# USCbiostats/bayesnetworks

Hardware: NVIDIA B200
Metric: edge_proposals_scored_per_sec (higher is better)
Workload: dtype f64

## Files before the change

### bayesnetworks_b200/csrc/chain_core.cuh

```cuda
#pragma once

#include "bn_common.cuh"
#include "rng_core.cuh"
#include "score_core.cuh"

namespace bn {

constexpr int WIN = 32;
constexpr int REPLAY_POS = 256;

constexpr int REC_LEN_MASK = 0xff;
constexpr int REC_TYPE = 1 << 8;
constexpr int REC_CYC = 1 << 9;
constexpr int REC_OVF = 1 << 10;
constexpr int REC_AG = 1 << 11;
constexpr int REC_ACC = 1 << 12;
constexpr int REC_NPD = 1 << 13;
constexpr int REC_FULLMANY = 1 << 14;
constexpr int REC_STALE = 1 << 15;
constexpr int REC_KK_SHIFT = 16;
constexpr int REC_NOSCORE = 1 << 23;
constexpr int REC_CLOSE = 1 << 24;
constexpr int WALK_STOP = 3 << 20;
constexpr int WALK_OVF = WALK_STOP | (1 << 24);
constexpr int WALK_STALE = WALK_STOP | (1 << 25);
constexpr int WALK_END = WALK_STOP | (1 << 26);

struct ChainParams {
  int P, max_par, W, Ws, n_samples;
  const double* C;
  int64_t ldc;
  const double* diag;
  ScoreConsts sc;
  const uint8_t* node_type;
  const uint8_t* sim_edge;
  int n_sim_edges;
  double phi, omega;
  int initial_network, drop, n_iter, output_every;
  int trace_capacity, moves_capacity;
  const int* prior_par;
  const int* prior_npar;
  int prior_stride;
  int g_chunks, g_lpr, g_rpp;
};

struct PipeLink;

struct ChainStart {
  int64_t iter;
  int valid;
  int te_m;
  int acc_add, acc_del;
};

struct ChainMem {
  int* par;
  int* npar;
  int* born;
  double* base;
  double* fac;
  double* rowbuf;
  uint32_t* anc;
  uint32_t* haspar;
  int* hp_list;
  int* scratch;
  volatile int* helper;
  int* t_iter; int* t_changed; int* t_movetype; double* t_gll;
  int* t_add; int* t_del; int* t_fn; int* t_fp;
  int* moves;
  int* edge_freq;
  double* dscore;
  int* npar_freq;
  int* npar_since;
  uint32_t* nver = nullptr;
  PipeLink* pipe = nullptr;
  int pipe_rank = 0;
  int pipe_debug = 0;
  const int* start_par = nullptr;
  const int* start_npar = nullptr;
  const ChainStart* start = nullptr;
  const double* base_in = nullptr;
};

struct ChainScalars {
  int64_t iter;
  int64_t read_pos;
  int valid;
  int te_m;
  int te_true, agree_true, n_haspar;
  int proposed[3], reject[3];
  int n_rows, n_moves, n_nonpd;
  int64_t valid_iters;
  int lane_prop[3], lane_rej[3], lane_nonpd, lane_valid;
  int64_t lane_bytes;
  int acc_add, acc_del;
  int gll_ok; double gll;
  int64_t alg_bytes;
  long long cyc[12];
  long long slots_sim;
  int win;
  int windows;
  int need_full;
  int anc_changed;
  int next_log;
  int status;
  int64_t pw_cur, pw_out_pos;
  int pw_out_seq, pw_out;
  int pw_seen;
  int pw_waits, pw_discards, pw_rebuilds;
  long long pw_cyc[6];
};

struct WindowSlots {
  int child[WIN], parent[WIN], pos[WIN], kk[WIN];
  int te_m[WIN], fp_m[WIN], fn_m[WIN];
  int64_t pos_after[WIN];
  double u_acc[WIN], new_score[WIN];
  signed char type[WIN], valid[WIN], do_check[WIN], accept[WIN], nonpd[WIN];
  int t_c[REPLAY_POS], t_j[REPLAY_POS], t_e[REPLAY_POS];
  int t_rec[REPLAY_POS];
  double t_score[REPLAY_POS];
  uint32_t t_full[REPLAY_POS];
  double t_lu[REPLAY_POS];
  int t_walk[2 * REPLAY_POS];
  int s_k[WIN];
};

BN_HD long long cycle_now() {
#if defined(__CUDA_ARCH__) && defined(BN_PHASE_CYCLES)
  return clock64();
#else
  return 0;
#endif
}

#if defined(BN_EMU_STATS) && !defined(__CUDA_ARCH__)
struct EmuStats { long del_total, del_trivial, del_desc, del_rounds, del_rows_eval, del_lost_bits, add_total, add_trivial, add_desc; };
inline EmuStats& emu_stats() { static EmuStats s = {}; return s; }
#define BN_STAT(x) x
#else
#define BN_STAT(x)
#endif

BN_HD bool test_bit(const uint32_t* row, int b) { return (row[b >> 5] >> (b & 31)) & 1u; }

BN_HD double prior_value(double phi, double omega, int dist, int total_edges) {
  return sub_rn(mul_rn(-phi, (double)dist), mul_rn(omega, (double)total_edges));
}

BN_HD int rank_below(const uint32_t* bits, int c) {
  const int l = Warp::lane(), cw = c >> 5;
  int cnt = 0;
  for (int w = l; w <= cw; w += Warp::NL) {
    uint32_t word = bits[w];
    if (w == cw) word &= (1u << (c & 31)) - 1u;
    cnt += popc32(word);
  }
  return Warp::sum(cnt);
}

BN_HD void hp_insert(ChainMem& m, int n_before, int c) {
  const int l = Warp::lane();
  const int idx = rank_below(m.haspar, c);
  for (int hi = n_before; hi > idx; hi -= Warp::NL) {
    const int i = hi - 1 - l;
    const int v = (i >= idx) ? m.hp_list[i] : 0;
    Warp::sync();
    if (i >= idx) m.hp_list[i + 1] = v;
    Warp::sync();
  }
  if (l == 0) m.hp_list[idx] = c;
  Warp::sync();
}
BN_HD void hp_remove(ChainMem& m, int n_before, int c) {
  const int l = Warp::lane();
  const int idx = rank_below(m.haspar, c);
  for (int lo = idx; lo < n_before - 1; lo += Warp::NL) {
    const int i = lo + l;
    const int v = (i < n_before - 1) ? m.hp_list[i + 1] : 0;
    Warp::sync();
    if (i < n_before - 1) m.hp_list[i] = v;
    Warp::sync();
  }
}

struct alignas(16) U4 { uint32_t x, y, z, w; };
BN_HD U4 or4(U4 a, U4 b) { U4 r; r.x = a.x | b.x; r.y = a.y | b.y; r.z = a.z | b.z; r.w = a.w | b.w; return r; }
BN_HD U4 andn4(U4 a, U4 b) { U4 r; r.x = a.x & ~b.x; r.y = a.y & ~b.y; r.z = a.z & ~b.z; r.w = a.w & ~b.w; return r; }
BN_HD U4 and4(U4 a, U4 b) { U4 r; r.x = a.x & b.x; r.y = a.y & b.y; r.z = a.z & b.z; r.w = a.w & b.w; return r; }
BN_HD bool nz4(U4 a) { return (a.x | a.y | a.z | a.w) != 0u; }
BN_HD bool ne4(U4 a, U4 b) { return ((a.x ^ b.x) | (a.y ^ b.y) | (a.z ^ b.z) | (a.w ^ b.w)) != 0u; }
BN_HD int popc4(U4 a) { return popc32(a.x) + popc32(a.y) + popc32(a.z) + popc32(a.w); }
BN_HD U4 with_bit(U4 v, int b) {
  const uint32_t m = 1u << (b & 31);
  const int w = b >> 5;
  v.x |= (w == 0) ? m : 0u; v.y |= (w == 1) ? m : 0u; v.z |= (w == 2) ? m : 0u; v.w |= (w == 3) ? m : 0u;
  return v;
}

struct RowGeom { int chunks, lpr, rpp; };
BN_HD void set_row_geom(ChainParams& p) {
  p.g_chunks = (p.W + 3) / 4;
  p.g_lpr = 1;
  while (p.g_lpr < p.g_chunks && p.g_lpr < Warp::NL) p.g_lpr <<= 1;
  p.g_rpp = Warp::NL / p.g_lpr;
}
BN_HD RowGeom row_geom(const ChainParams& p) {
  RowGeom g;
  g.chunks = p.g_chunks; g.lpr = p.g_lpr; g.rpp = p.g_rpp;
  return g;
}

BN_HD int group_sum(int v, int lpr) {
#if defined(__CUDA_ARCH__)
  for (int o = 1; o < lpr; o <<= 1) v += __shfl_xor_sync(0xffffffffu, v, o);
#else
  (void)lpr;
#endif
  return v;
}

BN_HD int atomic_fetch_inc(int* p) {
#if defined(__CUDA_ARCH__)
  return atomicAdd(p, 1);
#else
  return (*p)++;
#endif
}

BN_HD uint32_t atomic_or_u32(uint32_t* p, uint32_t v) {
#if defined(__CUDA_ARCH__)
  return atomicOr(p, v);
#else
  const uint32_t o = *p; *p = o | v; return o;
#endif
}

BN_HD int rows_per_part(int P, int nparts, int nl) {
  const int nblk = (P + nl - 1) / nl;
  return (nblk + nparts - 1) / nparts * nl;
}
BN_HD int scratch_words(int P, int nparts, int nl) {
  const int W = (P + 31) / 32;
  const int n = 2 * rows_per_part(P, nparts, nl) * nparts + 4 + (W + 3) / 4 * 4 + 3 * W + 4 + 1 + (W + 3) / 4 + 28;
  return (n + 3) / 4 * 4;
}

BN_HD int collect_desc_part(const ChainParams& p, const ChainMem& m, int c, int include_self, int* list,
                            int part, int nparts) {
  const int l = Warp::lane();
  const uint32_t Ws = (uint32_t)p.Ws, cb = (uint32_t)c & 31u;
  const uint32_t* col = m.anc + (c >> 5);
  const uint32_t lt = (1u << l) - 1u;
  int n = 0;
  const int step = nparts * Warp::NL;
  for (int d0 = part * Warp::NL; d0 < p.P; d0 += 4 * step) {
    int d[4], flag[4];
#pragma unroll
    for (int t = 0; t < 4; t++) {
      d[t] = d0 + t * step + l;
      flag[t] = 0;
      if (d[t] < p.P) flag[t] = ((col[(uint32_t)d[t] * Ws] >> cb) & 1u) & ((include_self || d[t] != c) ? 1u : 0u);
    }
#pragma unroll
    for (int t = 0; t < 4; t++) {
      const uint32_t mask = Warp::ballot(flag[t]);
      if (flag[t]) list[n + popc32(mask & lt)] = d[t];
      n += popc32(mask);
    }
  }
  Warp::sync();
  return n;
}

BN_HD void anc_add_part(const ChainParams& p, const ChainMem& m, int j, int c, int* list, int part, int nparts) {
  const RowGeom g = row_geom(p);
  const int l = Warp::lane(), sub = l / g.lpr, li = l % g.lpr;
  const int n = collect_desc_part(p, m, c, 1, list, part, nparts);
  BN_STAT(emu_stats().add_desc += n;)
  const U4* aj = (const U4*)(m.anc + (uint32_t)j * (uint32_t)p.Ws);
  if (g.chunks == 8 && Warp::NL == 32) {
    const int sub8 = l >> 3, li8 = l & 7;
    const U4 a = aj[li8];
    for (int r0 = sub8; r0 < n; r0 += 16) {
      U4* ad[4];
      U4 v[4];
#pragma unroll
      for (int t = 0; t < 4; t++) {
        const int r = (r0 + 4 * t < n) ? r0 + 4 * t : r0;
        ad[t] = (U4*)(m.anc + (uint32_t)list[r] * (uint32_t)p.Ws) + li8;
      }
#pragma unroll
      for (int t = 0; t < 4; t++) v[t] = *ad[t];
#pragma unroll
      for (int t = 0; t < 4; t++) *ad[t] = or4(v[t], a);
    }
  } else if (g.chunks <= g.lpr) {
    U4 a = {0u, 0u, 0u, 0u};
    if (li < g.chunks) {
      a = aj[li];
    }
    for (int r0 = 0; r0 < n; r0 += 4 * g.rpp) {
      U4* ad[4];
      U4 v[4];
#pragma unroll
      for (int t = 0; t < 4; t++) {
        const int r = r0 + t * g.rpp + sub;
        ad[t] = (r < n && li < g.chunks) ? (U4*)(m.anc + (uint32_t)list[r] * (uint32_t)p.Ws) + li : nullptr;
      }
#pragma unroll
      for (int t = 0; t < 4; t++) if (ad[t]) v[t] = *ad[t];
#pragma unroll
      for (int t = 0; t < 4; t++) if (ad[t]) *ad[t] = or4(v[t], a);
    }
  } else {
    for (int r0 = 0; r0 < n; r0 += g.rpp) {
      const int r = r0 + sub;
      if (r < n) {
        U4* ad = (U4*)(m.anc + (int64_t)list[r] * p.Ws);
        for (int ch = li; ch < g.chunks; ch += g.lpr) {
          ad[ch] = or4(ad[ch], aj[ch]);
        }
      }
    }
  }
  Warp::sync();
}

constexpr int HELPER_WARPS = 7;
enum { HELPER_EXIT = 0, HELPER_ANC_ADD = 1, HELPER_RECORDS = 2, HELPER_REPAIR = 3, HELPER_ANC_DEL = 4,
       HELPER_FILL_WH = 5, HELPER_PIPE_COPY = 6, HELPER_REPAIR_BATCH = 7 };
constexpr int HELPER_WORDS = 12;
#if defined(__CUDACC__)
__device__ __forceinline__ void cta_bar(int id) {
  asm volatile("bar.sync %0, %1;" ::"r"(id), "r"((HELPER_WARPS + 1) * 32) : "memory");
}
#endif
constexpr int PIPE_WIN = HELPER_WARPS * 32;
constexpr int PIPE_MQ = 64;
constexpr int PIPE_LOG = 128;
struct PipeLink {
  unsigned long long req;
  int req_exit;
  int pad0;
  unsigned long long rdy;
  int mq_tail;
  int pad1;
  alignas(16) int mq[PIPE_MQ][4];
  int log[PIPE_LOG];
};
constexpr int PIPE_MAX_NODES = 2048;
constexpr int LOG_NODE = 0xffffff, LOG_UNFULL = 1 << 24, LOG_ANC = 1 << 25, LOG_HP = 1 << 26;

#if defined(__CUDACC__)
__device__ __forceinline__ uint32_t smem_addr(const void* p) { return (uint32_t)__cvta_generic_to_shared(p); }
__device__ __forceinline__ uint32_t peer_addr(const void* p, int rank) {
  uint32_t r;
  asm volatile("mapa.shared::cluster.u32 %0, %1, %2;" : "=r"(r) : "r"(smem_addr(p)), "r"(rank));
  return r;
}
__device__ __forceinline__ void st_peer(uint32_t a, int v) {
  asm volatile("st.relaxed.cluster.shared::cluster.b32 [%0], %1;" ::"r"(a), "r"(v) : "memory");
}
__device__ __forceinline__ void st_peer64(uint32_t a, unsigned long long v) {
  asm volatile("st.relaxed.cluster.shared::cluster.b64 [%0], %1;" ::"r"(a), "l"(v) : "memory");
}
__device__ __forceinline__ void st_peer128(uint32_t a, int x, int y, int z, int w) {
  asm volatile("st.shared::cluster.v4.b32 [%0], {%1, %2, %3, %4};" ::"r"(a), "r"(x), "r"(y), "r"(z), "r"(w) : "memory");
}
__device__ __forceinline__ int ld_poll(const int* p) {
  int v;
  asm volatile("ld.volatile.shared.b32 %0, [%1];" : "=r"(v) : "r"(smem_addr(p)) : "memory");
  return v;
}
__device__ __forceinline__ unsigned long long ld_poll64(const unsigned long long* p) {
  unsigned long long v;
  asm volatile("ld.volatile.shared.b64 %0, [%1];" : "=l"(v) : "r"(smem_addr(p)) : "memory");
  return v;
}
__device__ __forceinline__ void ld_poll128(const int* p, int& x, int& y, int& z, int& w) {
  asm volatile("ld.volatile.shared.v4.b32 {%0, %1, %2, %3}, [%4];" : "=r"(x), "=r"(y), "=r"(z), "=r"(w) : "r"(smem_addr(p)) : "memory");
}
__device__ __forceinline__ int ld_peer(uint32_t a) {
  int v;
  asm volatile("ld.shared::cluster.b32 %0, [%1];" : "=r"(v) : "r"(a) : "memory");
  return v;
}
__device__ __forceinline__ long long ld_peer64(uint32_t a) {
  long long v;
  asm volatile("ld.shared::cluster.b64 %0, [%1];" : "=l"(v) : "r"(a) : "memory");
  return v;
}
__device__ __forceinline__ void cluster_sync_all() {
  asm volatile("barrier.cluster.arrive.release.aligned;\n\tbarrier.cluster.wait.acquire.aligned;" ::: "memory");
}

__device__ __forceinline__ void pipe_publish(const ChainMem& m, int n, int type, int c, int j, int del, int ag,
                                             double score, int flags) {
  PipeLink* lk = m.pipe;
  for (long long spins = 0; n - ld_poll(&lk->mq_tail) >= PIPE_MQ; spins++)
    if (spins > (1ll << 27)) { lk->pad1 = 92; break; }
  const long long sb = __double_as_longlong(score);
  st_peer128(peer_addr(&lk->mq[n % PIPE_MQ][0], 1), n + 1,
             c | (j << 11) | ((type - 1) << 22) | (del << 23) | (ag << 26) | ((n + 1) << 27),
             (int)(sb & 0xffffffffll), (int)(sb >> 32));
  lk->log[n % PIPE_LOG] = c | flags;
}
#endif

BN_HD void team_sync(const ChainMem& m) {
#if defined(__CUDA_ARCH__)
  if (m.helper) { cta_bar(3); return; }
#endif
  (void)m;
  Warp::sync();
}

BN_HD void anc_after_add(const ChainParams& p, ChainMem& m, int j, int c, int& m_anc_changed) {
  {
    const RowGeom g = row_geom(p);
    const U4* aj = (const U4*)(m.anc + (uint32_t)j * (uint32_t)p.Ws);
    const U4* ac = (const U4*)(m.anc + (uint32_t)c * (uint32_t)p.Ws);
    int news = 0;
    for (int ch = Warp::lane(); ch < g.chunks; ch += Warp::NL) news |= nz4(andn4(aj[ch], ac[ch])) ? 1 : 0;
    BN_STAT(emu_stats().add_total++;)
    if (Warp::ballot(news) == 0u) { BN_STAT(emu_stats().add_trivial++;) m_anc_changed = 0; return; }
  }
  m_anc_changed = 1;
#if defined(__CUDA_ARCH__)
  if (m.helper) {
    if (Warp::lane() == 0) { m.helper[8] = j; m.helper[9] = c; m.helper[0] = HELPER_ANC_ADD; }
    Warp::sync();
    cta_bar(1);
    if (!m.pipe) anc_add_part(p, m, j, c, m.scratch, 0, HELPER_WARPS + 1);
    cta_bar(2);
    return;
  }
#else
  anc_add_part(p, m, j, c, m.scratch, 0, 1);
#endif
}


struct Par8 { int q[8]; };
BN_HD Par8 load_par8(const ChainParams& p, const ChainMem& m, int d) {
  Par8 r;
  const int* pd = m.par + (int64_t)d * p.max_par;
  if (p.max_par == 8) {
    const U4 a = ((const U4*)pd)[0], b = ((const U4*)pd)[1];
    r.q[0] = (int)a.x; r.q[1] = (int)a.y; r.q[2] = (int)a.z; r.q[3] = (int)a.w;
    r.q[4] = (int)b.x; r.q[5] = (int)b.y; r.q[6] = (int)b.z; r.q[7] = (int)b.w;
  } else {
#pragma unroll
    for (int e = 0; e < 8; e++) r.q[e] = (e < p.max_par) ? pd[e] : -1;
  }
  return r;
}

struct DelLayout { int* lists; U4* L; uint32_t* dirty; volatile int* flags; int* nzc; int per; };
BN_HD DelLayout del_layout(const ChainParams& p, const ChainMem& m, int nparts) {
  DelLayout d;
  d.per = rows_per_part(p.P, nparts, Warp::NL);
  int off = (2 * d.per * nparts + 3) / 4 * 4;
  d.lists = m.scratch;
  d.L = (U4*)(m.scratch + off);
  off += (p.W + 3) / 4 * 4;
  d.dirty = (uint32_t*)(m.scratch + off);
  d.flags = (volatile int*)(d.dirty + 3 * p.W);
  d.nzc = (int*)(d.dirty + 3 * p.W + 4);
  return d;
}

BN_HD int anc_del_team(const ChainParams& p, const ChainMem& m, int c, int part, int nparts, long long* dbg = nullptr) {
  const int l = Warp::lane(), W = p.W, MP = p.max_par;
  const DelLayout lay = del_layout(p, m, nparts);
  int* list = lay.lists + (part < 0 ? 0 : part) * 2 * lay.per;
  int* list2 = list + lay.per;
  const long long td0 = cycle_now();
  const int n = part < 0 ? 0 : collect_desc_part(p, m, c, 0, list, part, nparts);
  BN_STAT(emu_stats().del_desc += n;)
  const uint32_t lt = (l == 31) ? 0x7fffffffu : ((1u << l) - 1u);
  const int nnz = lay.nzc[0];
  int lpr = 1;
  while (lpr < nnz && lpr < Warp::NL) lpr <<= 1;
  const int rpp = Warp::NL / lpr, sub = l / lpr, li = l % lpr;
  const uint32_t gm = (lpr >= 32 ? 0xffffffffu : ((1u << lpr) - 1u)) << (sub * lpr);
  for (int r0 = 0; r0 < n; r0 += rpp) {
    const int r = r0 + sub;
    if (r < n) {
      U4* ad = (U4*)(m.anc + (uint32_t)list[r] * (uint32_t)p.Ws);
      for (int t = li; t < nnz; t += lpr) {
        const int ch = lay.nzc[1 + t];
        ad[ch] = andn4(ad[ch], lay.L[ch]);
      }
    }
  }
  const long long td1 = cycle_now();
  team_sync(m);
  const long long td2 = cycle_now();
  if (dbg) { dbg[6] += td1 - td0; dbg[7] += td2 - td1; }
  int rounds_done = 0;
  for (int round = 0;; round++) {
    const long long tr0 = cycle_now();
    const uint32_t* dprev = lay.dirty + (round % 3) * W;
    uint32_t* dnext = lay.dirty + ((round + 1) % 3) * W;
    if (part <= 0 && (part < 0 || !m.pipe)) {
      uint32_t* dclr = lay.dirty + ((round + 2) % 3) * W;
      for (int w = l; w < W; w += Warp::NL) dclr[w] = 0u;
      if (l == 0) lay.flags[(round + 2) % 4] = 0;
    }
    const int* rows = list;
    int nt = n;
    if (round > 0) {
      rows = list2;
      nt = 0;
      for (int i0 = 0; i0 < n; i0 += Warp::NL) {
        const int i = i0 + l;
        const int d = (i < n) ? list[i] : -1;
        int touched = 0;
        if (d >= 0) {
          if (MP <= 8) {
            const Par8 pq = load_par8(p, m, d);
#pragma unroll
            for (int e = 0; e < 8; e++)
              if (pq.q[e] >= 0) touched |= (dprev[pq.q[e] >> 5] >> (pq.q[e] & 31)) & 1u;
          } else {
            const int kd = m.npar[d];
            const int* pd = m.par + (int64_t)d * MP;
            for (int e = 0; e < kd; e++) {
              const int q = pd[e];
              touched |= (dprev[q >> 5] >> (q & 31)) & 1u;
            }
          }
        }
        const uint32_t mask = Warp::ballot(touched);
        if (touched) list2[nt + popc32(mask & lt)] = d;
        nt += popc32(mask);
      }
      Warp::sync();
    }
    int any = 0;
    BN_STAT(emu_stats().del_rounds++; emu_stats().del_rows_eval += nt;)
    for (int r0 = 0; r0 < nt; r0 += rpp) {
      const int r = r0 + sub;
      int changed = 0, d = 0;
      if (r < nt) {
        d = rows[r];
        U4* ad = (U4*)(m.anc + (uint32_t)d * (uint32_t)p.Ws);
        for (int t = li; t < nnz; t += lpr) {
          const int ch = lay.nzc[1 + t];
          const U4 Lc = lay.L[ch];
          U4 v = {0u, 0u, 0u, 0u};
          if (MP <= 8) {
            const Par8 pq = load_par8(p, m, d);
#pragma unroll
            for (int e = 0; e < 8; e++) {
              const int q = pq.q[e];
              if (q >= 0) v = or4(v, ((const U4*)(m.anc + (uint32_t)q * (uint32_t)p.Ws))[ch]);
            }
          } else {
            const int kd = m.npar[d];
            const int* pd = m.par + (int64_t)d * MP;
            for (int e = 0; e < kd; e++) {
              const int q = pd[e];
              v = or4(v, ((const U4*)(m.anc + (int64_t)q * p.Ws))[ch]);
            }
          }
          const U4 cur = ad[ch];
          const U4 gain = andn4(and4(v, Lc), cur);
          if (nz4(gain)) { ad[ch] = or4(cur, gain); changed = 1; }
        }
      }
      const uint32_t mask = Warp::ballot(changed);
      if (r < nt && li == 0 && (mask & gm)) atomic_or_u32(&dnext[d >> 5], 1u << (d & 31));
      any |= (mask != 0u);
      Warp::sync();
    }
    if (any && l == 0) lay.flags[round % 4] = 1;
    const long long tr1 = cycle_now();
    team_sync(m);
    if (dbg) { dbg[8] += tr1 - tr0; dbg[11] += cycle_now() - tr1; }
    rounds_done++;
    if (lay.flags[round % 4] == 0) break;
  }
  return rounds_done;
}

BN_HD void anc_after_delete(const ChainParams& p, ChainMem& m, int c, int& m_anc_changed, long long* dbg = nullptr) {
  const RowGeom g = row_geom(p);
  const int l = Warp::lane();
  int nparts = 1;
#if defined(__CUDA_ARCH__)
  if (m.helper) nparts = m.pipe ? HELPER_WARPS : HELPER_WARPS + 1;
#endif
  const DelLayout lay = del_layout(p, m, nparts);
  {
    U4* ac = (U4*)(m.anc + (int64_t)c * p.Ws);
    const int* pc = m.par + (int64_t)c * p.max_par;
    const int kc = m.npar[c];
    int changed = 0;
    for (int ch = l; ch < g.chunks; ch += Warp::NL) {
      U4 v = {0u, 0u, 0u, 0u};
      if (ch == (c >> 7)) v = with_bit(v, c & 127);
      for (int e = 0; e < kc; e++) {
        const int q = pc[e];
        v = or4(v, ((const U4*)(m.anc + (int64_t)q * p.Ws))[ch]);
      }
      const U4 lost = andn4(ac[ch], v);
      lay.L[ch] = lost;
      if (nz4(lost)) { ac[ch] = v; changed = 1; }
    }
    BN_STAT(emu_stats().del_total++;)
    if (Warp::ballot(changed) == 0u) { BN_STAT(emu_stats().del_trivial++;) m_anc_changed = 0; return; }
  }
  m_anc_changed = 1;
  BN_STAT(for (int ch = 0; ch < g.chunks; ch++) emu_stats().del_lost_bits += popc4(lay.L[ch]);)
  for (int w = l; w < 3 * p.W + 4; w += Warp::NL) lay.dirty[w] = 0u;
  Warp::sync();
  {
    const uint32_t lt = (l == 31) ? 0x7fffffffu : ((1u << l) - 1u);
    int nnz = 0;
    for (int ch0 = 0; ch0 < g.chunks; ch0 += Warp::NL) {
      const int ch = ch0 + l;
      const int nz = (ch < g.chunks) && nz4(lay.L[ch]);
      const uint32_t mask = Warp::ballot(nz);
      if (nz) lay.nzc[1 + nnz + popc32(mask & lt)] = ch;
      nnz += popc32(mask);
    }
    if (l == 0) lay.nzc[0] = nnz;
    Warp::sync();
  }
#if defined(__CUDA_ARCH__)
  if (m.helper) {
    if (l == 0) { m.helper[9] = c; m.helper[0] = HELPER_ANC_DEL; }
    Warp::sync();
    cta_bar(1);
    anc_del_team(p, m, c, m.pipe ? -1 : 0, nparts, dbg);
    cta_bar(2);
    return;
  }
#else
  anc_del_team(p, m, c, 0, 1);
#endif
}

BN_HD void anc_reset(const ChainParams& p, ChainMem& m) {
  const int l = Warp::lane();
  for (int64_t i = l; i < (int64_t)p.P * p.Ws; i += Warp::NL) m.anc[i] = 0u;
  Warp::sync();
  for (int d = l; d < p.P; d += Warp::NL) m.anc[(int64_t)d * p.Ws + (d >> 5)] = 1u << (d & 31);
  Warp::sync();
}

BN_HD void anc_build_all(const ChainParams& p, ChainMem& m) {
  const RowGeom g = row_geom(p);
  const int l = Warp::lane(), P = p.P;
  anc_reset(p, m);
  for (int round = 0; round <= P; round++) {
    int changed = 0;
    for (int d = 0; d < P; d++) {
      const int kd = m.npar[d];
      if (kd == 0) continue;
      U4* ad = (U4*)(m.anc + (int64_t)d * p.Ws);
      const int* pd = m.par + (int64_t)d * p.max_par;
      for (int ch = l; ch < g.chunks; ch += Warp::NL) {
        U4 v = {0u, 0u, 0u, 0u};
        if (ch == (d >> 7)) v = with_bit(v, d & 127);
        for (int e = 0; e < kd; e++) {
          const int q = pd[e];
          v = or4(v, ((const U4*)(m.anc + (int64_t)q * p.Ws))[ch]);
        }
        if (ne4(v, ad[ch])) { ad[ch] = v; changed = 1; }
      }
      Warp::sync();
    }
    if (Warp::ballot(changed) == 0u) break;
  }
  Warp::sync();
}

template <int KMAX>
BN_HD double factor_current(const ChainParams& p, const ChainMem& m, int c) {
  const int MP = p.max_par, k = m.npar[c];
  double* F = m.fac + (int64_t)c * fac_stride(fac_mp(MP));
  if (k <= 8) {
    Parents8 S;
    const Par8 q = load_par8(p, m, c);
#pragma unroll
    for (int e = 0; e < 8; e++) S.s[e] = q.q[e];
    return factor_node8(p.C, p.ldc, c, S, k, p.sc, F, fac_mp(MP));
  }
  return factor_node(p.C, p.ldc, c, m.par + (int64_t)c * MP, k, p.sc, F, fac_mp(MP));
}

template <int KMAX>
BN_HD int64_t random_start(const ChainParams& p, ChainMem& m, RngStream& rng) {
  const int P = p.P, MP = p.max_par;
  int64_t pos = 0;
  int anc_changed = 0;
  for (int c = 0; c < P; c++) {
    if (p.node_type[c] == 1) continue;
    if (pos >= rng.gen_hi) rng_top_up(rng, pos);
    const int want = (int)(MP * rng.ubuf[pos & (RNG_CAP - 1)]);
    pos++;
    for (int slot = 0; slot < want; slot++) {
      int found = -1;
      for (int tries = 0; tries < 100 && found < 0; tries++) {
        if (pos >= rng.gen_hi) rng_top_up(rng, pos);
        const int j = (int)(P * rng.ubuf[pos & (RNG_CAP - 1)]);
        pos++;
        int ok = (j != c && p.node_type[j] != 2 && !test_bit(m.anc + (int64_t)j * p.Ws, c));
        for (int e = 0; e < slot; e++) if (m.par[(int64_t)c * MP + e] == j) ok = 0;
        if (ok) found = j;
      }
      if (found < 0) break;
      Warp::sync();
      if (Warp::lane() == 0) { m.par[(int64_t)c * MP + slot] = found; m.npar[c] = slot + 1; }
      Warp::sync();
      anc_after_add(p, m, found, c, anc_changed);
    }
  }
  return pos;
}

template <int KMAX>
BN_HD void chain_init(const ChainParams& p, ChainMem& m, ChainScalars& s, RngStream& rng) {
  const int l = Warp::lane(), P = p.P, MP = p.max_par;
  const bool given = m.start_par != nullptr;
  const int64_t it0 = m.start ? m.start->iter : 0;
  const int counted_from = (m.start && it0 > p.drop) ? (int)it0 : p.drop;
  for (int64_t i = l; i < (int64_t)P * MP; i += Warp::NL) {
    const int c = (int)(i / MP), e = (int)(i % MP);
    m.par[i] = given ? m.start_par[i]
                     : (p.initial_network == 0 && e < p.prior_npar[c]) ? p.prior_par[(int64_t)c * p.prior_stride + e] : -1;
    if (m.born) m.born[i] = counted_from;
  }
  if (m.npar_freq)
    for (int i = l; i < P; i += Warp::NL) m.npar_since[i] = counted_from;
  for (int i = l; i < P; i += Warp::NL) m.npar[i] = given ? m.start_npar[i] : (p.initial_network == 0) ? p.prior_npar[i] : 0;
  for (int w = l; w < p.W; w += Warp::NL) m.haspar[w] = 0u;
  if (m.nver)
    for (int i = l; i < P; i += Warp::NL) m.nver[i] = 0u;
  Warp::sync();
  int64_t start_pos = 0;
  const bool random = !given && p.initial_network == 1;
  if (random) {
    anc_reset(p, m);
    start_pos = random_start<KMAX>(p, m, rng);
  }
  if (l == 0) {
    int te = 0, ag = 0, nh = 0;
    for (int c = 0; c < P; c++) {
      const int k = m.npar[c];
      if (k) { m.haspar[c >> 5] |= 1u << (c & 31); m.hp_list[nh] = c; nh++; }
      for (int e = 0; e < k; e++) {
        te++;
        if (p.sim_edge[(int64_t)m.par[(int64_t)c * MP + e] + (int64_t)c * P]) ag++;
      }
    }
    s.te_true = te; s.agree_true = ag; s.n_haspar = nh;
  }
  s.te_true = Warp::shfl(s.te_true, 0);
  s.agree_true = Warp::shfl(s.agree_true, 0);
  s.n_haspar = Warp::shfl(s.n_haspar, 0);
  Warp::sync();
  if (random) {  }
  else if (s.te_true > 0) anc_build_all(p, m);
  else anc_reset(p, m);
  s.n_nonpd = 0;
  for (int c = l; c < P; c += Warp::NL) {
    if (m.base_in) {
      m.base[c] = m.base_in[c];
    } else if (KMAX <= 8) {
      Parents8 S;
      const int k = m.npar[c];
#pragma unroll
      for (int e = 0; e < 8; e++) S.s[e] = (e < k) ? m.par[(int64_t)c * MP + e] : c;
      m.base[c] = score_set8(p.C, p.ldc, c, S, k, p.n_samples);
    } else {
      m.base[c] = factor_current<KMAX>(p, m, c);
    }
  }
  Warp::sync();
  s.iter = it0; s.read_pos = start_pos;
  s.valid = m.start ? m.start->valid : 1;
  s.te_m = m.start ? m.start->te_m : 0;
  for (int t = 0; t < 3; t++) { s.proposed[t] = 0; s.reject[t] = 0; s.lane_prop[t] = 0; s.lane_rej[t] = 0; }
  s.lane_nonpd = 0; s.lane_valid = 0; s.lane_bytes = 0;
  s.acc_add = m.start ? m.start->acc_add : 0; s.acc_del = m.start ? m.start->acc_del : 0;
  s.n_rows = 0; s.n_moves = 0; s.valid_iters = 0; s.alg_bytes = 0;
  s.gll_ok = 0; s.gll = 0.0;
// ... 631 lines not shown
template <int KMAX, bool PIPE = false>
BN_HD void team_records(const ChainParams& p, const ChainMem& m, const RoundCtx& rc, const double* ubuf,
                        WindowSlots& ws) {
#if defined(__CUDA_ARCH__)
  if (m.helper) {
    helper_post(m, HELPER_RECORDS, rc);
    cta_bar(1);
    if constexpr (!PIPE) build_record<KMAX>(p, m, rc, ubuf, ws, Warp::lane());
    cta_bar(2);
    return;
  }
#else
  for (int slot = Warp::lane(); slot < REPLAY_POS; slot += Warp::NL) build_record<KMAX>(p, m, rc, ubuf, ws, slot);
  Warp::sync();
#endif
}

BN_HD void team_repair(const ChainParams& p, const ChainMem& m, WindowSlots& ws, int c, int unfull, int retest,
                       int from) {
#if defined(__CUDA_ARCH__)
  if (m.helper) {
    if (Warp::lane() == 0) {
      m.helper[8] = from; m.helper[9] = c; m.helper[11] = unfull; m.helper[7] = retest;
      m.helper[0] = HELPER_REPAIR;
    }
    Warp::sync();
    cta_bar(1);
    if (!m.pipe) repair_record(p, m, ws, Warp::lane(), c, unfull, retest, from);
    cta_bar(2);
  }
#else
  for (int slot = Warp::lane(); slot < REPLAY_POS; slot += Warp::NL)
    repair_record(p, m, ws, slot, c, unfull, retest, from);
  Warp::sync();
#endif
}

BN_HD void write_row_vals(const ChainParams& p, ChainMem& m, ChainScalars& s, int64_t it, int child,
                          int type, int fn, int fp, int additions, int deletions) {
  if (!s.gll_ok) { s.gll = sum_base(p, m); s.gll_ok = 1; }
  if (s.n_rows < p.trace_capacity) {
    if (Warp::lane() == 0) {
      const int r = s.n_rows;
      m.t_iter[r] = (int)it;
      m.t_changed[r] = child;
      m.t_movetype[r] = type;
      m.t_gll[r] = s.gll;
      m.t_add[r] = additions;
      m.t_del[r] = deletions;
      m.t_fn[r] = fn;
      m.t_fp[r] = fp;
    }
    s.n_rows++;
  }
}
BN_HD void write_row(const ChainParams& p, ChainMem& m, ChainScalars& s, int64_t it,
                     const WindowSlots& ws, int i, int additions, int deletions) {
  write_row_vals(p, m, s, it, ws.child[i], ws.type[i], ws.fn_m[i], ws.fp_m[i], additions, deletions);
}

template <int KMAX>
BN_HD void apply_move_vals(const ChainParams& p, ChainMem& m, ChainScalars& s, int64_t it, int type, int c,
                           int j, int del, double new_score, int ag, const double* newrow) {
  const int MP = p.max_par, l = Warp::lane();
#if defined(__CUDA_ARCH__)
  if (m.pipe) {
    const int kk0 = m.npar[c];
    bool bad = (type == 1) ? (kk0 >= MP) : (del < 0 || del >= kk0 || m.par[(int64_t)c * MP + del] != j);
    if (type == 1) for (int e = 0; e < kk0 && e < MP; e++) bad |= m.par[(int64_t)c * MP + e] == j;
    if (bad) { s.status = 95; return; }
  }
#endif
  int* pc = m.par + (int64_t)c * MP;
  int* bc = m.born ? m.born + (int64_t)c * MP : nullptr;
  const int k = m.npar[c];
  double* F = KMAX > 8 ? m.fac + (int64_t)c * fac_stride(fac_mp(MP)) : nullptr;
#if defined(__CUDA_ARCH__)
  D2 rv, rd, rr;
  rv.x = rv.y = rd.x = rd.y = rr.x = rr.y = 0.0;
  if (KMAX > 8 && type == 1 && newrow) {
    if (2 * l < k) rv = ld2_l2(newrow + 2 * l);
    rd = ld2_l2(newrow + row_tail(fac_mp(MP)));
    rr = ld2_l2(newrow + row_tail(fac_mp(MP)) + 2);
  }
#endif
  const long long tq0 = cycle_now();
  const int64_t first_counted = (it > p.drop) ? it : p.drop;
#if defined(__CUDA_ARCH__)
  const bool publish = m.pipe && m.pipe_rank == 0 && m.pipe_debug != 2;
  const long long tp0 = cycle_now();
  if (publish && l == 0)
    pipe_publish(m, s.n_moves, type, c, j, type == 2 ? del : 0, ag, new_score,
                 ((type == 2 && k == MP) ? LOG_UNFULL : 0) | ((type == 1 ? k == 0 : k == 1) ? LOG_HP : 0));
  s.pw_cyc[5] += cycle_now() - tp0;
#endif
  Warp::sync();
  if (l == 0 && m.npar_freq) {
    const int64_t cnt = first_counted - m.npar_since[c];
    if (cnt > 0) m.npar_freq[(int64_t)c * (MP + 1) + k] += (int)cnt;
    m.npar_since[c] = (int)first_counted;
  }
  if (type == 1) {
    if (l == 0) {
      pc[k] = j; m.npar[c] = k + 1;
      if (m.edge_freq) bc[k] = (int)first_counted;
      m.base[c] = new_score;
      if (KMAX > 8 && !newrow) factor_current<KMAX>(p, m, c);
    }
    if (k == 0) {
      Warp::sync();
      hp_insert(m, s.n_haspar, c);
      if (l == 0) m.haspar[c >> 5] |= 1u << (c & 31);
      s.n_haspar++;
    }
    s.te_true++; s.agree_true += ag;
    Warp::sync();
    const long long tq1 = cycle_now();
    anc_after_add(p, m, j, c, s.anc_changed);
    (void)tq1;
  } else {
    if (l == 0) {
      if (m.edge_freq) {
        const int64_t cnt = first_counted - bc[del];
        if (cnt > 0) m.edge_freq[(int64_t)j + (int64_t)c * p.P] += (int)cnt;
      }
      for (int e = del; e + 1 < k; e++) pc[e] = pc[e + 1];
      if (m.edge_freq)
        for (int e = del; e + 1 < k; e++) bc[e] = bc[e + 1];
      pc[k - 1] = -1;
      m.npar[c] = k - 1;
      if (KMAX > 8) {
        const double rss_old = F[fac_tail(fac_mp(MP))];
        m.base[c] = (rss_old == rss_old) ? factor_downdate<KMAX>(F, k, del, p.sc, fac_mp(MP)) : factor_current<KMAX>(p, m, c);
      } else {
        m.base[c] = new_score;
      }
    }
    if (k == 1) {
      Warp::sync();
      hp_remove(m, s.n_haspar, c);
      if (l == 0) m.haspar[c >> 5] &= ~(1u << (c & 31));
      s.n_haspar--;
    }
    s.te_true--; s.agree_true -= ag;
    Warp::sync();
    const long long tq1 = cycle_now();
#if defined(BN_PHASE_CYCLES)
    anc_after_delete(p, m, c, s.anc_changed, s.cyc);
#else
    anc_after_delete(p, m, c, s.anc_changed);
#endif
    s.cyc[9] += tq1 - tq0; s.cyc[10] += cycle_now() - tq1;
  }
  if (KMAX > 8 && type == 1 && newrow) {
    const int mp = fac_mp(MP);
#if defined(__CUDA_ARCH__)
    const double r = rsqrt_f64(rd.x);
    if (2 * l <= k) {
      if (2 * l == k) rv.x = r;
      if (2 * l + 1 == k) rv.y = r;
      *(D2*)(F + fac_row(k) + 2 * l) = rv;
    }
    if (l == 0) { F[fac_zoff(mp) + k] = rd.y * r; F[fac_tail(mp)] = rr.x; }
#else
    const double r = rsqrt_f64(newrow[row_tail(mp)]);
    for (int t = 0; t < k; t++) F[fac_row(k) + t] = newrow[t];
    F[fac_row(k) + k] = r;
    F[fac_zoff(mp) + k] = newrow[row_tail(mp) + 1] * r; F[fac_tail(mp)] = newrow[row_tail(mp) + 2];
#endif
  }
  if (m.nver) {
    if (l == 0) m.nver[c]++;
  } else if (m.dscore) {
    double* dc = m.dscore + (uint32_t)c * (uint32_t)MP;
    for (int e = l; e < MP; e += Warp::NL) dc[e] = nan_sentinel();
  }
#if defined(__CUDA_ARCH__)
  if (publish && l == 0 && s.anc_changed) m.pipe->log[s.n_moves % PIPE_LOG] |= LOG_ANC;
#endif
  if (s.n_moves < p.moves_capacity) {
    if (l == 0) {
      int* mv = m.moves + (int64_t)s.n_moves * 4;
      mv[0] = (int)it; mv[1] = type; mv[2] = c; mv[3] = j;
    }
  }
  s.n_moves++;
  s.gll_ok = 0;
  Warp::sync();
}

template <int KMAX>
BN_HD void apply_move(const ChainParams& p, ChainMem& m, ChainScalars& s, int64_t it,
                      const WindowSlots& ws, int i) {
  const int ag = p.sim_edge[(int64_t)ws.parent[i] + (int64_t)ws.child[i] * p.P] ? 1 : 0;
  apply_move_vals<KMAX>(p, m, s, it, ws.type[i], ws.child[i], ws.parent[i], ws.pos[i], ws.new_score[i], ag, nullptr);
}

template <int KMAX>
BN_HD void commit(const ChainParams& p, ChainMem& m, ChainScalars& s, const WindowSlots& ws,
                  int ncommit) {
  const int l = Warp::lane();
  for (int i0 = 0; i0 < ncommit; i0 += Warp::NL) {
    const int i = i0 + l;
    const bool in = i < ncommit;
    const int64_t it = s.iter + i;
    const bool valid = in && ws.valid[in ? i : 0];
    const int type = in ? ws.type[i] : 0;
    const bool counted = valid && it >= p.drop;
    const bool acc = valid && ws.accept[in ? i : 0];
    const uint32_t m_valid = Warp::ballot(valid);
    const uint32_t m_inval = Warp::ballot(in && !valid);
    const uint32_t m_p1 = Warp::ballot(counted && type == 1);
    const uint32_t m_p2 = Warp::ballot(counted && type == 2);
    const uint32_t m_r1 = Warp::ballot(counted && type == 1 && !acc);
    const uint32_t m_r2 = Warp::ballot(counted && type == 2 && !acc);
    const uint32_t m_npd = Warp::ballot(valid && ws.nonpd[in ? i : 0]);
    const uint32_t m_acc = Warp::ballot(acc);
    const uint32_t m_log = Warp::ballot(valid && ((int)it % p.output_every == 0));
    const int kk = valid ? ws.kk[i] : 0;
    const int bytes = Warp::sum(valid ? 4 * (kk + 1) * (kk + 2) + 8 : 0);
    uint32_t lg = m_log & ~m_acc;
    while (lg) {
      const int b = ffs32(lg) - 1;
      lg &= lg - 1;
      const uint32_t upto = (b == 31) ? 0xffffffffu : ((2u << b) - 1u);
      (void)upto;
      write_row(p, m, s, s.iter + i0 + b, ws, i0 + b, s.acc_add, s.acc_del);
    }
    s.valid_iters += popc32(m_valid);
    s.alg_bytes += bytes;
    s.proposed[1] += popc32(m_p1); s.proposed[2] += popc32(m_p2);
    s.reject[0] += popc32(m_inval);
    s.reject[1] += popc32(m_r1); s.reject[2] += popc32(m_r2);
    s.n_nonpd += popc32(m_npd);
    if (m_acc) {
      const int b = ffs32(m_acc) - 1;
      const long long ta = cycle_now();
      apply_move<KMAX>(p, m, s, s.iter + i0 + b, ws, i0 + b);
      const long long dt = cycle_now() - ta;
      s.cyc[ws.type[i0 + b] == 1 ? 4 : 5] += dt;
      s.cyc[3] -= dt;
      if (s.iter + i0 + b >= p.drop) { if (ws.type[i0 + b] == 1) s.acc_add++; else s.acc_del++; }
      if (m_log & m_acc) write_row(p, m, s, s.iter + i0 + b, ws, i0 + b, s.acc_add, s.acc_del);
    }
  }
  const int last = ncommit - 1;
  s.valid = ws.valid[last];
  s.te_m = ws.te_m[last];
  s.read_pos = ws.pos_after[last];
  s.iter += ncommit;
  Warp::sync();
}

template <int KMAX>
BN_HD int round_epoch(const ChainParams& p, ChainMem& m, ChainScalars& s, const WindowSlots& ws, int64_t round_pos,
                      int* k_io, int want, int* stop, int* accepted, int* acc_c, int* acc_type) {
  const int l = Warp::lane();
  int k = *k_io, v = s.valid, n = 0, myk = 0, myvalid = 0, acc = 0, k_acc = 0;
  *stop = 0;
  while (n < want) {
    const int w = ws.t_walk[k];
    const int f = w >> (16 + v);
    if (f & 0x14) {
      if (f & 0x10) { *stop = w; break; }
      if (l == n) { myk = k; myvalid = 1; }
      acc = 1; k_acc = k;
      k += (w >> (v << 3)) & 0xff;
      v = 1;
      n++;
      break;
    }
    if (l == n) { myk = k; myvalid = f & 1; }
    k += (w >> (v << 3)) & 0xff;
    v = f & 1;
    n++;
  }
  *accepted = acc;
  if (n == 0) return 0;
  const long long tc = cycle_now();
  const int last = n - 1;
  const bool in = l < n;
  const int rec = in ? ws.t_rec[myk] : 0;
  const int type = (rec & REC_TYPE) ? 2 : 1;
  const bool valid = in && myvalid;
  const int it0 = (int)s.iter, it = it0 + l;
  const bool counted = valid && it >= p.drop;
  const bool is_acc = acc && l == last;
  s.lane_prop[1] += (counted && type == 1) ? 1 : 0;
  s.lane_prop[2] += (counted && type == 2) ? 1 : 0;
  s.lane_rej[1] += (counted && type == 1 && !is_acc) ? 1 : 0;
  s.lane_rej[2] += (counted && type == 2 && !is_acc) ? 1 : 0;
  s.lane_rej[0] += (in && !myvalid) ? 1 : 0;
  if (valid) {
    const int kk = rec >> REC_KK_SHIFT;
    s.lane_valid++;
    s.lane_bytes += 4 * (kk + 1) * (kk + 2) + 8;
    if (rec & REC_NPD) s.lane_nonpd++;
  }
  int log_acc = 0, fn_acc = 0, fp_acc = 0;
  if (s.next_log < it0 + n) {
    const int ag = (rec & REC_AG) ? 1 : 0;
    const int te_m = valid ? s.te_true + (type == 1 ? 1 : -1) : s.te_true;
    const int ag_new = valid ? s.agree_true + (type == 1 ? ag : -ag) : s.agree_true;
    const int fp_m = te_m - ag_new, fn_m = p.n_sim_edges - ag_new;
    const int child = in ? ws.t_c[myk] : 0;
    do {
// ... 357 lines not shown
```

Baseline: 124.7 million.

## Replace iterative ancestor-deletion fixpoint with inflow-set single-pass repair

Ancestor-matrix maintenance after an edge delete no longer runs an iterative dirty-row fixpoint with repeated rounds and team syncs. It first sets each descendant's lost bits from parents that do not reach the deleted-edge child and records rows with inflow. It then prunes rows whose lost ancestors are fully explained, and finally ORs inflow-set ancestor rows into each descendant using a warp reduction. The aim is to remove the multi-round convergence loop and its barriers, at the cost of more per-row parent reads and a serial per-row final pass. Correctness depends on the closure argument, which is why a host-side check hook was added.

```diff
diff --git a/bayesnetworks_b200/csrc/chain_core.cuh b/bayesnetworks_b200/csrc/chain_core.cuh
--- a/bayesnetworks_b200/csrc/chain_core.cuh
+++ b/bayesnetworks_b200/csrc/chain_core.cuh
@@ -135,11 +135,14 @@
 }
 
 #if defined(BN_EMU_STATS) && !defined(__CUDA_ARCH__)
-struct EmuStats { long del_total, del_trivial, del_desc, del_rounds, del_rows_eval, del_lost_bits, add_total, add_trivial, add_desc; };
+struct EmuStats { long del_total, del_trivial, del_desc, del_inflow, del_inflow_hits, del_lost_bits, add_total, add_trivial, add_desc; };
 inline EmuStats& emu_stats() { static EmuStats s = {}; return s; }
 #define BN_STAT(x) x
 #else
 #define BN_STAT(x)
+#endif
+#if defined(BN_ANC_CHECK) && !defined(__CUDA_ARCH__)
+void anc_check_hook(const ChainParams& p, const ChainMem& m);
 #endif
 
 BN_HD bool test_bit(const uint32_t* row, int b) { return (row[b >> 5] >> (b & 31)) & 1u; }
@@ -191,6 +194,13 @@
 BN_HD bool nz4(U4 a) { return (a.x | a.y | a.z | a.w) != 0u; }
 BN_HD bool ne4(U4 a, U4 b) { return ((a.x ^ b.x) | (a.y ^ b.y) | (a.z ^ b.z) | (a.w ^ b.w)) != 0u; }
 BN_HD int popc4(U4 a) { return popc32(a.x) + popc32(a.y) + popc32(a.z) + popc32(a.w); }
+BN_HD U4 warp_or4(U4 v) {
+#if defined(__CUDA_ARCH__)
+  v.x = __reduce_or_sync(0xffffffffu, v.x); v.y = __reduce_or_sync(0xffffffffu, v.y);
+  v.z = __reduce_or_sync(0xffffffffu, v.z); v.w = __reduce_or_sync(0xffffffffu, v.w);
+#endif
+  return v;
+}
 BN_HD U4 with_bit(U4 v, int b) {
   const uint32_t m = 1u << (b & 31);
   const int w = b >> 5;
@@ -228,6 +238,13 @@
 #endif
 }
 
+BN_HD uint32_t atomic_and_u32(uint32_t* p, uint32_t v) {
+#if defined(__CUDA_ARCH__)
+  return atomicAnd(p, v);
+#else
+  const uint32_t o = *p; *p = o & v; return o;
+#endif
+}
 BN_HD uint32_t atomic_or_u32(uint32_t* p, uint32_t v) {
 #if defined(__CUDA_ARCH__)
   return atomicOr(p, v);
@@ -242,7 +259,7 @@
 }
 BN_HD int scratch_words(int P, int nparts, int nl) {
   const int W = (P + 31) / 32;
-  const int n = 2 * rows_per_part(P, nparts, nl) * nparts + 4 + (W + 3) / 4 * 4 + 3 * W + 4 + 1 + (W + 3) / 4 + 28;
+  const int n = (rows_per_part(P, nparts, nl) * nparts + 3) / 4 * 4 + (W + 3) / 4 * 4 + W + (1 + W) + (1 + (W + 3) / 4);
   return (n + 3) / 4 * 4;
 }
 
@@ -457,133 +474,134 @@
   return r;
 }
 
-struct DelLayout { int* lists; U4* L; uint32_t* dirty; volatile int* flags; int* nzc; int per; };
+struct DelLayout { int* lists; U4* L; uint32_t* S; int* nzs; int* nzc; int per; };
 BN_HD DelLayout del_layout(const ChainParams& p, const ChainMem& m, int nparts) {
   DelLayout d;
   d.per = rows_per_part(p.P, nparts, Warp::NL);
-  int off = (2 * d.per * nparts + 3) / 4 * 4;
+  int off = (d.per * nparts + 3) / 4 * 4;
   d.lists = m.scratch;
   d.L = (U4*)(m.scratch + off);
   off += (p.W + 3) / 4 * 4;
-  d.dirty = (uint32_t*)(m.scratch + off);
-  d.flags = (volatile int*)(d.dirty + 3 * p.W);
-  d.nzc = (int*)(d.dirty + 3 * p.W + 4);
+  d.S = (uint32_t*)(m.scratch + off);
+  d.nzs = m.scratch + off + p.W;
+  d.nzc = d.nzs + 1 + p.W;
   return d;
 }
 
-BN_HD int anc_del_team(const ChainParams& p, const ChainMem& m, int c, int part, int nparts, long long* dbg = nullptr) {
-  const int l = Warp::lane(), W = p.W, MP = p.max_par;
+BN_HD void anc_del_team(const ChainParams& p, const ChainMem& m, int c, int part, int nparts, long long* dbg = nullptr) {
+  const int l = Warp::lane(), MP = p.max_par;
   const DelLayout lay = del_layout(p, m, nparts);
-  int* list = lay.lists + (part < 0 ? 0 : part) * 2 * lay.per;
-  int* list2 = list + lay.per;
+  int* list = lay.lists + (part < 0 ? 0 : part) * lay.per;
   const long long td0 = cycle_now();
   const int n = part < 0 ? 0 : collect_desc_part(p, m, c, 0, list, part, nparts);
   BN_STAT(emu_stats().del_desc += n;)
-  const uint32_t lt = (l == 31) ? 0x7fffffffu : ((1u << l) - 1u);
   const int nnz = lay.nzc[0];
   int lpr = 1;
   while (lpr < nnz && lpr < Warp::NL) lpr <<= 1;
   const int rpp = Warp::NL / lpr, sub = l / lpr, li = l % lpr;
   const uint32_t gm = (lpr >= 32 ? 0xffffffffu : ((1u << lpr) - 1u)) << (sub * lpr);
+  const uint32_t cw = (uint32_t)c >> 5, cb = (uint32_t)c & 31u;
   for (int r0 = 0; r0 < n; r0 += rpp) {
     const int r = r0 + sub;
+    int e = 0, inflow = 0;
     if (r < n) {
-      U4* ad = (U4*)(m.anc + (uint32_t)list[r] * (uint32_t)p.Ws);
+      e = list[r];
+      U4* ae = (U4*)(m.anc + (uint32_t)e * (uint32_t)p.Ws);
       for (int t = li; t < nnz; t += lpr) {
         const int ch = lay.nzc[1 + t];
-        ad[ch] = andn4(ad[ch], lay.L[ch]);
-      }
-    }
+        const U4 Lc = lay.L[ch];
+        U4 v = {0u, 0u, 0u, 0u};
+        if (MP <= 8) {
+          const Par8 pq = load_par8(p, m, e);
+#pragma unroll
+          for (int k = 0; k < 8; k++) {
+            const int q = pq.q[k];
+            if (q >= 0) {
+              const uint32_t* aq = m.anc + (uint32_t)q * (uint32_t)p.Ws;
+              if (!((aq[cw] >> cb) & 1u)) v = or4(v, ((const U4*)aq)[ch]);
+            }
+          }
+        } else {
+          const int kd = m.npar[e];
+          const int* pd = m.par + (int64_t)e * MP;
+#pragma unroll 1
+          for (int k = 0; k < kd; k++) {
+            const uint32_t* aq = m.anc + (uint32_t)pd[k] * (uint32_t)p.Ws;
+            if (!((aq[cw] >> cb) & 1u)) v = or4(v, ((const U4*)aq)[ch]);
+          }
+        }
+        const U4 in = and4(v, Lc);
+        ae[ch] = or4(andn4(ae[ch], Lc), in);
+        inflow |= nz4(in) ? 1 : 0;
+      }
+    }
+    const uint32_t mask = Warp::ballot(inflow);
+    if (r < n && li == 0 && (mask & gm) && atomic_or_u32(&lay.S[e >> 5], 1u << (e & 31)) == 0u)
+      lay.nzs[1 + atomic_fetch_inc(&lay.nzs[0])] = e >> 5;
   }
   const long long td1 = cycle_now();
   team_sync(m);
-  const long long td2 = cycle_now();
-  if (dbg) { dbg[6] += td1 - td0; dbg[7] += td2 - td1; }
-  int rounds_done = 0;
-  for (int round = 0;; round++) {
-    const long long tr0 = cycle_now();
-    const uint32_t* dprev = lay.dirty + (round % 3) * W;
-    uint32_t* dnext = lay.dirty + ((round + 1) % 3) * W;
-    if (part <= 0 && (part < 0 || !m.pipe)) {
-      uint32_t* dclr = lay.dirty + ((round + 2) % 3) * W;
-      for (int w = l; w < W; w += Warp::NL) dclr[w] = 0u;
-      if (l == 0) lay.flags[(round + 2) % 4] = 0;
-    }
-    const int* rows = list;
-    int nt = n;
-    if (round > 0) {
-      rows = list2;
-      nt = 0;
-      for (int i0 = 0; i0 < n; i0 += Warp::NL) {
-        const int i = i0 + l;
-        const int d = (i < n) ? list[i] : -1;
-        int touched = 0;
-        if (d >= 0) {
-          if (MP <= 8) {
-            const Par8 pq = load_par8(p, m, d);
+  for (int r0 = 0; r0 < n; r0 += rpp) {
+    const int r = r0 + sub;
+    int e = 0, extra = 0;
+    const bool ins = r < n && test_bit(lay.S, e = list[r]);
+    if (ins) {
+      const U4* ae = (const U4*)(m.anc + (uint32_t)e * (uint32_t)p.Ws);
+      for (int t = li; t < nnz; t += lpr) {
+        const int ch = lay.nzc[1 + t];
+        const U4 Lc = lay.L[ch];
+        U4 v = {0u, 0u, 0u, 0u};
+        if (MP <= 8) {
+          const Par8 pq = load_par8(p, m, e);
 #pragma unroll
-            for (int e = 0; e < 8; e++)
-              if (pq.q[e] >= 0) touched |= (dprev[pq.q[e] >> 5] >> (pq.q[e] & 31)) & 1u;
-          } else {
-            const int kd = m.npar[d];
-            const int* pd = m.par + (int64_t)d * MP;
-            for (int e = 0; e < kd; e++) {
-              const int q = pd[e];
-              touched |= (dprev[q >> 5] >> (q & 31)) & 1u;
+          for (int k = 0; k < 8; k++) {
+            const int q = pq.q[k];
+            if (q >= 0) {
+              const uint32_t* aq = m.anc + (uint32_t)q * (uint32_t)p.Ws;
+              if ((aq[cw] >> cb) & 1u) v = or4(v, ((const U4*)aq)[ch]);
             }
           }
+        } else {
+          const int kd = m.npar[e];
+          const int* pd = m.par + (int64_t)e * MP;
+#pragma unroll 1
+          for (int k = 0; k < kd; k++) {
+            const uint32_t* aq = m.anc + (uint32_t)pd[k] * (uint32_t)p.Ws;
+            if ((aq[cw] >> cb) & 1u) v = or4(v, ((const U4*)aq)[ch]);
+          }
         }
-        const uint32_t mask = Warp::ballot(touched);
-        if (touched) list2[nt + popc32(mask & lt)] = d;
-        nt += popc32(mask);
-      }
-      Warp::sync();
-    }
-    int any = 0;
-    BN_STAT(emu_stats().del_rounds++; emu_stats().del_rows_eval += nt;)
-    for (int r0 = 0; r0 < nt; r0 += rpp) {
-      const int r = r0 + sub;
-      int changed = 0, d = 0;
-      if (r < nt) {
-        d = rows[r];
-        U4* ad = (U4*)(m.anc + (uint32_t)d * (uint32_t)p.Ws);
-        for (int t = li; t < nnz; t += lpr) {
-          const int ch = lay.nzc[1 + t];
-          const U4 Lc = lay.L[ch];
-          U4 v = {0u, 0u, 0u, 0u};
-          if (MP <= 8) {
-            const Par8 pq = load_par8(p, m, d);
-#pragma unroll
-            for (int e = 0; e < 8; e++) {
-              const int q = pq.q[e];
-              if (q >= 0) v = or4(v, ((const U4*)(m.anc + (uint32_t)q * (uint32_t)p.Ws))[ch]);
-            }
-          } else {
-            const int kd = m.npar[d];
-            const int* pd = m.par + (int64_t)d * MP;
-            for (int e = 0; e < kd; e++) {
-              const int q = pd[e];
-              v = or4(v, ((const U4*)(m.anc + (int64_t)q * p.Ws))[ch]);
-            }
-          }
-          const U4 cur = ad[ch];
-          const U4 gain = andn4(and4(v, Lc), cur);
-          if (nz4(gain)) { ad[ch] = or4(cur, gain); changed = 1; }
+        extra |= nz4(andn4(and4(ae[ch], Lc), v)) ? 1 : 0;
+      }
+    }
+    const uint32_t mask = Warp::ballot(extra);
+    if (ins && li == 0 && !(mask & gm)) atomic_and_u32(&lay.S[e >> 5], ~(1u << (e & 31)));
+  }
+  team_sync(m);
+  const long long td2 = cycle_now();
+  const int ns = lay.nzs[0];
+  BN_STAT(for (int k = 0; k < ns; k++) emu_stats().del_inflow += popc32(lay.S[lay.nzs[1 + k]]);)
+  for (int r = 0; ns > 0 && r < n; r++) {
+    uint32_t* ad = m.anc + (uint32_t)list[r] * (uint32_t)p.Ws;
+    int hit = 0;
+    for (int k = l; k < ns; k += Warp::NL) hit |= (ad[lay.nzs[1 + k]] & lay.S[lay.nzs[1 + k]]) != 0u;
+    if (Warp::ballot(hit) == 0u) continue;
+    for (int t = 0; t < nnz; t++) {
+      const int ch = lay.nzc[1 + t];
+      U4 acc = {0u, 0u, 0u, 0u};
+      for (int k = l; k < ns; k += Warp::NL) {
+        const int w = lay.nzs[1 + k];
+        uint32_t x = ad[w] & lay.S[w];
+        BN_STAT(if (t == 0) emu_stats().del_inflow_hits += popc32(x);)
+        for (; x; x &= x - 1u) {
+          const uint32_t e = ((uint32_t)w << 5) + (uint32_t)(ffs32(x) - 1);
+          acc = or4(acc, ((const U4*)(m.anc + e * (uint32_t)p.Ws))[ch]);
         }
       }
-      const uint32_t mask = Warp::ballot(changed);
-      if (r < nt && li == 0 && (mask & gm)) atomic_or_u32(&dnext[d >> 5], 1u << (d & 31));
-      any |= (mask != 0u);
-      Warp::sync();
-    }
-    if (any && l == 0) lay.flags[round % 4] = 1;
-    const long long tr1 = cycle_now();
-    team_sync(m);
-    if (dbg) { dbg[8] += tr1 - tr0; dbg[11] += cycle_now() - tr1; }
-    rounds_done++;
-    if (lay.flags[round % 4] == 0) break;
-  }
-  return rounds_done;
+      acc = warp_or4(acc);
+      if (l == 0) ((U4*)ad)[ch] = or4(((U4*)ad)[ch], and4(acc, lay.L[ch]));
+    }
+  }
+  if (dbg) { dbg[6] += td1 - td0; dbg[7] += td2 - td1; dbg[8] += cycle_now() - td2; }
 }
 
 BN_HD void anc_after_delete(const ChainParams& p, ChainMem& m, int c, int& m_anc_changed, long long* dbg = nullptr) {
@@ -615,8 +633,8 @@
   }
   m_anc_changed = 1;
   BN_STAT(for (int ch = 0; ch < g.chunks; ch++) emu_stats().del_lost_bits += popc4(lay.L[ch]);)
-  for (int w = l; w < 3 * p.W + 4; w += Warp::NL) lay.dirty[w] = 0u;
-  Warp::sync();
+  for (int w = l; w < p.W; w += Warp::NL) lay.S[w] = 0u;
+  if (l == 0) lay.nzs[0] = 0;
   {
     const uint32_t lt = (l == 31) ? 0x7fffffffu : ((1u << l) - 1u);
     int nnz = 0;
@@ -636,7 +654,9 @@
     Warp::sync();
     cta_bar(1);
     anc_del_team(p, m, c, m.pipe ? -1 : 0, nparts, dbg);
+    const long long tb = cycle_now();
     cta_bar(2);
+    if (dbg) dbg[11] += cycle_now() - tb;
     return;
   }
 #else
@@ -1574,6 +1594,9 @@
 #endif
     s.cyc[9] += tq1 - tq0; s.cyc[10] += cycle_now() - tq1;
   }
+#if defined(BN_ANC_CHECK) && !defined(__CUDA_ARCH__)
+  anc_check_hook(p, m);
+#endif
   if (KMAX > 8 && type == 1 && newrow) {
     const int mp = fac_mp(MP);
 #if defined(__CUDA_ARCH__)
```

Measured after the change: 79.41 million (median of 6 runs). 36.3% lower.
